# bjack205/rsLQR

Measured on AMD Instinct MI355X. Metric: LQR solves/sec (nx=12,nu=4,N=256,batch=1024 per GPU), higher is better.
Workload: dtype f64; 1 GPU; nx=12 nu=4 N=256 batch=1024 per GPU, fp64, factor+solve per step; parallelism=batch-sharded x1, no data-path collective, ranks_seen=1, flags=0, schedule=reduced-fused2

## Files before the change

### rslqr_amd/csrc/hip_context.hpp

```cpp
#pragma once
#include <hip/hip_runtime.h>

#include <cstdio>
#include <cstdlib>
#include <cstring>
#include <string>
#include <vector>

#include "ndlqr.h"
#include "ndlqr_hip.h"

#include "kernels_common.hpp"

int ndlqr_hip_fail(const char* what, hipError_t e);
struct NdlqrHipCtx;
int ndlqr_hip_ensure_F(NdlqrHipCtx* c);
#define HIP_TRY(expr)                                                  \
  do {                                                                 \
    hipError_t e_ = (expr);                                            \
    if (e_ != hipSuccess) return ndlqr_hip_fail(#expr, e_);            \
  } while (0)


enum { SLOT_LEAF = 0, SLOT_SEP, SLOT_SCHUR, SLOT_BOUNDARY, SLOT_APPLY, SLOT_BOTTOM, SLOT_UPPER, SLOT_TOP, SLOT_COUNT };

struct PendingEvent {
  int slot;
  hipEvent_t start, stop;
};

struct CapturedChain {
  hipGraphExec_t exec = nullptr;
  unsigned flags = 0;
  hipStream_t stream = nullptr;
  unsigned apply = 0;
  bool rec_complete = false;
  bool rec_compact = false;
  const char* schedule = "none";
  void reset() {
    if (exec) (void)hipGraphExecDestroy(exec);
    exec = nullptr;
  }
};

struct BufferSet {
  double* rec = nullptr;
  double* red = nullptr;
  size_t red_bytes = 0;
  double* ytop = nullptr;
  double* z = nullptr;
  double* rhs = nullptr;
  double* xfer = nullptr;
  int* tree_cnt = nullptr;
  int* h_fail = nullptr;
  hipStream_t stream = nullptr;
  hipEvent_t ev_start = nullptr, ev_stop = nullptr;
  unsigned long long rhs_gen[4] = {};
  CapturedChain graph;
  bool ready = false;
};

struct KnotSlice {
  int knot0 = 0, nknots = 0;
  unsigned blocks = 7u;
  bool valid(int N, unsigned allowed) const {
    return knot0 >= 0 && nknots > 0 && knot0 + nknots <= N && (blocks & 7u) && !(blocks & ~allowed);
  }
  size_t width(const ndlqr::Dims& u) const {
    return ((blocks & 1u) ? u.n : 0) + ((blocks & 2u) ? u.n : 0) + ((blocks & 4u) ? u.m : 0);
  }
  size_t doubles(const ndlqr::Dims& u) const { return nknots > 0 ? width(u) * nknots : (size_t)u.rows * u.N - u.m; }
};

struct NdlqrHipCtx {
  ndlqr::Dims d = {};
  ndlqr::Dims du = {};
  bool padded = false;
  double* pad_stage = nullptr;
  size_t pad_stage_cap = 0;
  int device = 0;
  unsigned flags = 0;
  bool own_stream = true;
  double* AB = nullptr;
  double* QR = nullptr;
  double* F = nullptr;
  int rowbcast = -1;
  int tree = -1;
  int fuse2 = -1;
  BufferSet set[2];
  int cur = 0;
  int latest = 0;
  int pipeline = 2;
  unsigned solve_count = 0;
  bool state_dirty = false;
  int fail_base = 0;
  int* info = nullptr;
  const char* schedule = "none";
  double* kkt_out = nullptr;
  size_t multi_cap = 0;
  double *multi_rhs = nullptr, *multi_z = nullptr, *multi_zsep = nullptr, *multi_fsum = nullptr, *multi_ytop = nullptr,
         *multi_in = nullptr, *multi_out = nullptr;
  double* sep_scratch = nullptr;
  double* h_stage[2] = {};
  bool no_top = false;
  int top_levels = 3;
  bool no_mfma = false;
  bool rec_complete = false;
  bool rec_compact = false;
  int sep_threads = 0;
  hipEvent_t ev_step[2] = {};
  unsigned step_count = 0;
  hipEvent_t ev_inputs = nullptr;
  unsigned long long rhs_latest[4] = {};
  KnotSlice sel;
  int apply_blk0 = 0, apply_nblk = 0;
  bool z_partial = false;
  bool z_invalid = false;
  int z_blk0 = 0, z_nblk = 0;
  int step_set[2] = {};
  double* h_io = nullptr;
  CapturedChain staged;
  bool timing_pending = false;
  double last_ms = 0;
  int last_failures = 0;
  bool fact_valid = false;
  double* adj_rhs = nullptr;
  double* adj_z = nullptr;
  double* adj_save = nullptr;
  double* grad_stage = nullptr;
  size_t grad_stage_cap = 0;
  unsigned long long soln_gen = 0, adj_gen = 0;
  bool inputs_replaced = false;
  double *box_lo = nullptr, *box_hi = nullptr, *box_v = nullptr, *box_y = nullptr, *box_z = nullptr, *box_qr_save = nullptr;
  double* box_rhs[2] = {};
  double* box_resid = nullptr;
  unsigned char* box_mask = nullptr;
  int *box_status = nullptr, *box_iters = nullptr, *box_word = nullptr;
  int* h_box_word = nullptr;
  bool box_shared = false, box_have_bounds = false, box_have_vy = false;
  size_t box_bstride = 0;
  bool box_fact = false;
  double box_rho = 0.0;
  unsigned box_flags = 0;
  bool box_rec_complete = false, box_rec_compact = false, box_fact_valid = false;
  const char* box_schedule = "none";
  unsigned long long box_soln_gen = 0, abox_gen = 0;
  unsigned char* abox_code = nullptr;
  double *abox_v = nullptr, *abox_y = nullptr, *abox_resid = nullptr;
  double* abox_rhs[2] = {};
  int *abox_status = nullptr, *abox_iters = nullptr, *abox_word = nullptr;
  unsigned long long factor_count = 0;
  std::vector<PendingEvent> pending;
  std::vector<hipEvent_t> event_pool;
  double slot_ms[SLOT_COUNT] = {};
  int slot_launches[SLOT_COUNT] = {};
};

static inline hipEvent_t take_event(NdlqrHipCtx* c) {
  if (!c->event_pool.empty()) {
    hipEvent_t ev = c->event_pool.back();
    c->event_pool.pop_back();
    return ev;
  }
  hipEvent_t ev = nullptr;
  (void)hipEventCreate(&ev);
  return ev;
}

struct ScopedSlot {
  NdlqrHipCtx* c;
// ... 14 lines not shown
```

### rslqr_amd/csrc/kernels_rowbcast.hpp

```cpp
#pragma once
#include "kernels_dpp.hpp"
#include "kernels_small.hpp"

namespace ndlqr {

template <int K, bool NEG>
__device__ __forceinline__ void fmac_bc4(double& a0, double& a1, double& a2, double& a3, const double x0, const double x1,
                                         const double x2, const double x3, const double y) {
  if constexpr (NEG)
    asm volatile("v_fmac_f64_dpp %0, -%4, %8 row_newbcast:%9 row_mask:0xf bank_mask:0xf\n\t"
                 "v_fmac_f64_dpp %1, -%5, %8 row_newbcast:%9 row_mask:0xf bank_mask:0xf\n\t"
                 "v_fmac_f64_dpp %2, -%6, %8 row_newbcast:%9 row_mask:0xf bank_mask:0xf\n\t"
                 "v_fmac_f64_dpp %3, -%7, %8 row_newbcast:%9 row_mask:0xf bank_mask:0xf"
                 : "+v"(a0), "+v"(a1), "+v"(a2), "+v"(a3) : "v"(x0), "v"(x1), "v"(x2), "v"(x3), "v"(y), "n"(K));
  else
    asm volatile("v_fmac_f64_dpp %0, %4, %8 row_newbcast:%9 row_mask:0xf bank_mask:0xf\n\t"
                 "v_fmac_f64_dpp %1, %5, %8 row_newbcast:%9 row_mask:0xf bank_mask:0xf\n\t"
                 "v_fmac_f64_dpp %2, %6, %8 row_newbcast:%9 row_mask:0xf bank_mask:0xf\n\t"
                 "v_fmac_f64_dpp %3, %7, %8 row_newbcast:%9 row_mask:0xf bank_mask:0xf"
                 : "+v"(a0), "+v"(a1), "+v"(a2), "+v"(a3) : "v"(x0), "v"(x1), "v"(x2), "v"(x3), "v"(y), "n"(K));
}

template <int KD, int NC, bool INIT, bool NEG = false, int NA, int NB>
__device__ __forceinline__ void rb_mul(const double (&A)[NA], double (&B)[NB], double (&out)[NC]) {
// ... 324 lines not shown
    if (hasA && rowlane) {
#pragma unroll
      for (int c = 0; c < NX; ++c)
        if (c >= i) atomicAdd(sA.DR() + c * (c + 1) / 2 + i, G[c]);
      atomicAdd(sA.gR() + i, gv);
    }
    rb_mul<NX, NX, true>(RaTt, Xb, G);
    if (hasA && hasB && rowlane) {
      if (leftchild) {
#pragma unroll
        for (int c = 0; c < NX; ++c) sB.CA()[c * NX + i] = G[c];
      } else {
        store_row<NX>(sA.CB() + i * NX, G);
      }
    }
    rb_mul<NX, NX, true>(RbTt, Xb, G);
    gv = rb_mulv<NX>(RbTt, xz);
    if (hasB && rowlane) {
#pragma unroll
      for (int c = 0; c < NX; ++c)
        if (c >= i) atomicAdd(sB.DL() + c * (c + 1) / 2 + i, G[c]);
      atomicAdd(sB.gL() + i, gv);
    }
  }
}

template <int NX>
__device__ __forceinline__ void backsub_top_body(const Dims& d, const int b, const int t,
                                                 const double* __restrict__ recs, double* __restrict__ ytop,
                                                 double* ytop_lds, const int bp, const double* zsep) {
  constexpr int NN = NX * NX, REC = 2 * NN + NX;
  const int N = d.N, K = d.K;
  const int br = bp >= 0 ? bp : b;
  for (int L = K - 1; L >= 3; --L) {
    const int T = 2 << L, nsep = N >> (L + 1);
    for (int it = t; it < nsep * NX; it += 256) {
      const int q = it / NX, r = it - q * NX;
      const int base = q * T, s = base + (T >> 1) - 1;
      const double* rc = recs + ((size_t)br * N + s) * REC;
      double acc = zsep ? zsep[((size_t)b * N + s) * NX + r] : rc[2 * NN + r];
      if (base > 0) {
        double f[NX];
        load_row<NX>(rc + r * NX, f);
        const double* y = ytop_lds + ((base - 1) >> 3) * NX;
#pragma unroll
        for (int c = 0; c < NX; ++c) acc = fma(-f[c], y[c], acc);
      }
      if (base + T < N) {
        double f[NX];
        load_row<NX>(rc + NN + r * NX, f);
        const double* y = ytop_lds + ((base + T - 1) >> 3) * NX;
#pragma unroll
        for (int c = 0; c < NX; ++c) acc = fma(-f[c], y[c], acc);
      }
      ytop_lds[(s >> 3) * NX + r] = acc;
    }
    __syncthreads();
  }
  double* out = ytop + (size_t)b * (N >> 3) * NX;
  for (int e = t; e < ((N >> 3) - 1) * NX; e += 256) out[e] = ytop_lds[e];
}

template <int NX>
__global__ __launch_bounds__(256) void rb_backsub_top(Dims d, const double* __restrict__ recs, double* __restrict__ ytop) {
  extern __shared__ double ytop_lds[];
  backsub_top_body<NX>(d, blockIdx.x, threadIdx.x, recs, ytop, ytop_lds);
}

template <int NX, int NU>
struct alignas(16) RbBacksubLds {
  static constexpr int W = NX + NU, ROWS = 2 * NX + NU, NN = NX * NX, REC = 2 * NN + NX, R0 = NX * (NX + 1) / 2;
  static constexpr int R0P = (R0 + 1) / 2 * 2;
  static constexpr int WP = RbKnot<NX, NU>::WP;
  double ab[8][NX * WP];
  double rec0[4][R0P];
  double rec1[3][REC + (REC & 1)];
  double ys[9][NX];
  double qs[8][W];
  double rs[8][ROWS];
  double dots[8][NX];
  double vs[4][NX];
};

template <int NX, int NU, bool MULTI = false>
__global__ __launch_bounds__(256) void rb_backsub(Dims d, const double* __restrict__ AB, const double* __restrict__ QR,
                                                  const double* __restrict__ rhs, const double* __restrict__ recs,
                                                  const double* __restrict__ ytop, double* __restrict__ z,
                                                  const int nprob = 0, const double* __restrict__ zsep = nullptr) {
  using Lds = RbBacksubLds<NX, NU>;
  constexpr int W = NX + NU, ROWS = 2 * NX + NU, NN = NX * NX, REC = 2 * NN + NX, KPB = 8, WP = Lds::WP;
  constexpr int R0 = Lds::R0;
  static_assert(9 * NX <= 256 && KPB * ROWS <= 256, "thread roles fit the workgroup");
  __shared__ Lds lds;
  const int N = d.N, b = blockIdx.y, first = (blockIdx.x + d.xoff) * KPB;
  const int bp = MULTI ? b % nprob : b;
  auto sep_slot = [&](int s) -> int { return s < first ? 7 : (s >= first + 7 ? 8 : s - first); };
  const int t = threadIdx.x;

  {
    const double* abm = AB + ((size_t)bp * N + first) * NX * W;
    const double* rc0 = recs + ((size_t)bp * N + first) * REC;
    constexpr int NA = KPB * NX * W / 2, IA = (NA + 255) / 256;
    constexpr bool WIDE = NX % 2 == 0 && R0 % 2 == 0;
    constexpr int G = WIDE ? 2 : 1;
    constexpr int N0 = 4 * R0 / G, I0 = (N0 + 255) / 256, N1 = 3 * REC / G, I1 = (N1 + 255) / 256;
    constexpr int NQ = KPB * W, NR = KPB * ROWS;
    static_assert(NQ <= 256 && NR <= 256, "one load per thread for the vectors");
    static_assert((KPB * NX * W) % 2 == 0, "eight knots of [A | B] are whole 16-byte words");
    constexpr int KW = NX * W / 2;
    constexpr bool BYKNOT = (NX * W) % 2 == 0 && KW % 32 == 0;
    constexpr int JA = BYKNOT ? KW / 32 : IA;
    double2 ta[JA];
    double t0[I0][G], t1[I1][G];
#pragma unroll
    for (int it = 0; it < JA; ++it) {
      if constexpr (BYKNOT) {
        ta[it] = reinterpret_cast<const double2*>(abm)[(t >> 5) * KW + (t & 31) + 32 * it];
      } else {
        const int e = t + 256 * it;
        ta[it] = reinterpret_cast<const double2*>(abm)[e < NA ? e : NA - 1];
      }
    }
#pragma unroll
    for (int it = 0; it < I0; ++it) {
      const int e = t + 256 * it, ec = e < N0 ? e : N0 - 1, j = ec / (R0 / G), w_ = ec - j * (R0 / G);
      const double* src = rc0 + (size_t)(2 * j) * REC + G * w_;
      if constexpr (WIDE) { const double2 v = *reinterpret_cast<const double2*>(src); t0[it][0] = v.x; t0[it][1] = v.y; }
      else t0[it][0] = *src;
    }
#pragma unroll
    for (int it = 0; it < I1; ++it) {
      const int e = t + 256 * it, ec = e < N1 ? e : N1 - 1, j = ec / (REC / G), w_ = ec - j * (REC / G);
      const double* src = rc0 + (size_t)(2 * j + 1) * REC + G * w_;
      if constexpr (WIDE) { const double2 v = *reinterpret_cast<const double2*>(src); t1[it][0] = v.x; t1[it][1] = v.y; }
      else t1[it][0] = *src;
    }
    const double tq = QR[((size_t)bp * N + first) * W + (t < NQ ? t : NQ - 1)];
    const double tr = rhs[((size_t)b * N + first) * ROWS + (t < NR ? t : NR - 1)];
    double tz = 0.0;
    if constexpr (MULTI) {
      const int e = t < 3 * NX ? t : 3 * NX - 1, j = e / NX;
      tz = zsep[((size_t)b * N + first + 2 * j + 1) * NX + (e - j * NX)];
    }
    double ty = 0.0;
    if (t < 2 * NX) {
      const int sx = t < NX ? first - 1 : first + 7;
      if (sx >= 0 && sx < N - 1) ty = ytop[((size_t)b * (N >> 3) + (sx >> 3)) * NX + (t < NX ? t : t - NX)];
    }
#pragma unroll
    for (int it = 0; it < JA; ++it) {
      if constexpr (BYKNOT) {
        const int w_ = 2 * ((t & 31) + 32 * it), row = w_ / W, c = w_ - row * W;
        *reinterpret_cast<double2*>(&lds.ab[t >> 5][row * WP + c]) = ta[it];
      } else {
        const int e = t + 256 * it, ec = e < NA ? e : NA - 1;
#pragma unroll
        for (int h = 0; h < 2; ++h) {
          const int ed = 2 * ec + h, kn = ed / (NX * W), w_ = ed - kn * NX * W;
          const int row = w_ / W, c = w_ - row * W;
          lds.ab[kn][row * WP + c] = h ? ta[it].y : ta[it].x;
        }
      }
    }
#pragma unroll
    for (int it = 0; it < I0; ++it) {
      const int e = t + 256 * it, ec = e < N0 ? e : N0 - 1, j = ec / (R0 / G), w_ = ec - j * (R0 / G);
#pragma unroll
      for (int h = 0; h < G; ++h) lds.rec0[j][G * w_ + h] = t0[it][h];
    }
#pragma unroll
    for (int it = 0; it < I1; ++it) {
// ... 37 lines not shown
      const double* rc = lds.rec1[q >> 1];
      double a = rc[2 * NN + r];
      if (hasA) {
#pragma unroll
        for (int c = 0; c < NX; ++c) a = fma(-rc[r * NX + c], lds.ys[slotA][c], a);
      }
      if (hasB) {
#pragma unroll
        for (int c = 0; c < NX; ++c) a = fma(-rc[NN + r * NX + c], lds.ys[slotB][c], a);
      }
      lds.ys[q][r] = a;
    }
    __syncthreads();
  }
  const bool odd_state = out_thread && (kn & 1) && rr >= NX && rr < 2 * NX;
  double dot = 0.0;
  if (odd_state) {
    if (needs_ab) dot = ab_dot(lds.ys[sep_slot(i)]);
    lds.dots[kn][rr - NX] = dot;
  }
  __syncthreads();
  if (sep_thread && l == 0) {
    const int k = s - first;
    const bool fst = s == 0;
    const double* arow = lds.ab[k] + r * WP;
    double v = 0.0;
#pragma unroll
    for (int c = 0; c < W; ++c) {
      const double wq = lds.qs[k][c];
      double zh;
      if (c < NX) zh = fst ? -lds.rs[k][c] : (lds.rs[k][NX + c] + (hasA ? lds.ys[slotA][c] : 0.0)) * wq;
      else zh = lds.rs[k][NX + c] * wq;
      v = fma(arow[c], zh, v);
    }
    const double q1 = lds.qs[k + 1][r];
    v -= lds.rs[k + 1][r] + (lds.rs[k + 1][NX + r] - lds.dots[k + 1][r]) * q1;
    lds.vs[k >> 1][r] = v;
  }
  __syncthreads();
  if (t < 64) {
    const int j = t >> 4, r15 = t & 15, rc = r15 < NX ? r15 : NX - 1;
    const double* Lp = lds.rec0[j];
    const double dinv = 1.0 / Lp[rc * (rc + 1) / 2 + rc];
    double lrow[NX], lcol[NX];
#pragma unroll
    for (int c = 0; c < NX; ++c) {
      const double lo = Lp[rc * (rc + 1) / 2 + (c < rc ? c : rc)];
      const double up = Lp[(c > rc ? c : rc) * ((c > rc ? c : rc) + 1) / 2 + rc];
      lrow[c] = (c < r15 && r15 < NX) ? lo : 0.0;
      lcol[c] = (c > r15 && r15 < NX) ? up : 0.0;
    }
    double x = lds.vs[j][rc];
    sfor<NX>([&](auto cc) {
      constexpr int c = decltype(cc)::value;
      double xs = x * dinv;
      dpp_fence(xs);
      x = fma(-lrow[c], row_bc<c>(xs), x);
    });
    x = x * dinv;
    sfor<NX>([&](auto cc) {
      constexpr int c = NX - 1 - decltype(cc)::value;
      double xs = x * dinv;
      dpp_fence(xs);
      x = fma(-lcol[c], row_bc<c>(xs), x);
    });
    if (r15 < NX) lds.ys[2 * j][r15] = x * dinv;
  }
  __syncthreads();

  if (!out_thread) return;
  const double rv = lds.rs[kn][rr];
  double out;
  const double* yi = lds.ys[sep_slot(i < N - 1 ? i : i - 1)];
  const double* yp = lds.ys[sep_slot(i > 0 ? i - 1 : 0)];
  if (needs_ab && !odd_state) dot = ab_dot(yi);
  if (lam) {
    out = (i == 0) ? fma(-QR[(size_t)bp * N * W + rr], rv, -lds.rs[0][NX + rr]) + dot : yp[rr];
  } else if (rr < 2 * NX) {
    out = (i == 0) ? -lds.rs[0][rr - NX] : (rv - dot + yp[rr - NX]) * lds.qs[kn][rr - NX];
  } else {
    out = (i == N - 1) ? rv : (rv - dot) * lds.qs[kn][rr - NX];
  }
  z[((size_t)b * N + i) * ROWS + rr] = out;
}

template <int NX>
__device__ __forceinline__ double rb_llt_solve(double x, const double (&lrow)[NX], const double (&lcol)[NX], const double dinv) {
  sfor<NX>([&](auto cc) {
    constexpr int c = decltype(cc)::value;
    double xs = x * dinv;
    dpp_fence(xs);
    x = fma(-lrow[c], row_bc<c>(xs), x);
  });
  x = x * dinv;
  sfor<NX>([&](auto cc) {
    constexpr int c = NX - 1 - decltype(cc)::value;
    double xs = x * dinv;
    dpp_fence(xs);
    x = fma(-lcol[c], row_bc<c>(xs), x);
  });
  return x * dinv;
}

template <int NX, int NU>
struct alignas(16) RbForwardLds {
  static constexpr int W = NX + NU, ROWS = 2 * NX + NU, NN = NX * NX, REC = 2 * NN + NX, R0 = NX * (NX + 1) / 2;
  static constexpr int R0P = (R0 + 1) / 2 * 2, WP = RbKnot<NX, NU>::WP;
  double ab[8][NX * WP];
  double rec0[4][R0P];
  double l1[3][NN];
  double f1[3][2 * NN];
  double qs[8][W];
  double rs[8][ROWS];
  double bt[7][NX];
  double zs[4][NX];
  double gl[7][NX], gr[7][NX];
  double outl[3][NX], outr[3][NX];
};

template <int NX, int NU, bool MULTI = false>
__global__ __launch_bounds__(256) void rb_forward(Dims d, const double* __restrict__ AB, const double* __restrict__ QR,
                                                  const double* __restrict__ rhs, double* __restrict__ recs,
                                                  double* __restrict__ fsum, const int nprob = 0,
                                                  double* __restrict__ zsep = nullptr) {
  using Lds = RbForwardLds<NX, NU>;
  constexpr int W = NX + NU, ROWS = 2 * NX + NU, NN = NX * NX, REC = 2 * NN + NX, KPB = 8, WP = Lds::WP, R0 = Lds::R0;
  static_assert(7 * NX <= 256 && KPB * ROWS <= 256 && KPB * W <= 256, "thread roles fit the workgroup");
  __shared__ Lds lds;
  const int N = d.N, b = blockIdx.y, first = blockIdx.x * KPB, t = threadIdx.x;
  const int bp = MULTI ? b % nprob : b;
  {
    const double* abm = AB + ((size_t)bp * N + first) * NX * W;
    const double* rc0 = recs + ((size_t)bp * N + first) * REC;
    constexpr bool WIDE = NX % 2 == 0 && R0 % 2 == 0 && (NX * W) % 2 == 0;
    constexpr int G = WIDE ? 2 : 1;
    constexpr int NA = KPB * NX * W / G, IA = (NA + 255) / 256;
    constexpr int N0 = 4 * R0 / G, I0 = (N0 + 255) / 256, NL = 3 * NN / G, IL = (NL + 255) / 256;
    constexpr int NF = 3 * 2 * NN / G, IF = (NF + 255) / 256;
    double ta[IA][G], t0[I0][G], tl[IL][G], tf[IF][G];
    auto ld = [](const double* src, double (&dst)[G]) {
      if constexpr (WIDE) { const double2 v = *reinterpret_cast<const double2*>(src); dst[0] = v.x; dst[1] = v.y; }
      else dst[0] = *src;
    };
#pragma unroll
    for (int it = 0; it < IA; ++it) { const int e = t + 256 * it, ec = e < NA ? e : NA - 1; ld(abm + G * ec, ta[it]); }
#pragma unroll
    for (int it = 0; it < I0; ++it) {
      const int e = t + 256 * it, ec = e < N0 ? e : N0 - 1, j = ec / (R0 / G), w_ = ec - j * (R0 / G);
      ld(rc0 + (size_t)(2 * j) * REC + G * w_, t0[it]);
    }
#pragma unroll
    for (int it = 0; it < IL; ++it) {
      const int e = t + 256 * it, ec = e < NL ? e : NL - 1, j = ec / (NN / G), w_ = ec - j * (NN / G);
      ld(rc0 + (size_t)(2 * j) * REC + rb_lrec_offset<NX>() + G * w_, tl[it]);
    }
#pragma unroll
    for (int it = 0; it < IF; ++it) {
      const int e = t + 256 * it, ec = e < NF ? e : NF - 1, j = ec / (2 * NN / G), w_ = ec - j * (2 * NN / G);
      ld(rc0 + (size_t)(2 * j + 1) * REC + G * w_, tf[it]);
    }
    const double tq = QR[((size_t)bp * N + first) * W + (t < KPB * W ? t : KPB * W - 1)];
    const double tr = rhs[((size_t)b * N + first) * ROWS + (t < KPB * ROWS ? t : KPB * ROWS - 1)];
#pragma unroll
    for (int it = 0; it < IA; ++it) {
      const int e = t + 256 * it, ec = e < NA ? e : NA - 1;
#pragma unroll
// ... 200 lines not shown
```

### rslqr_amd/csrc/launch_small.hpp

```cpp
#pragma once
#include "hip_context.hpp"
#include "kernels_leaf.hpp"
#include "kernels_small.hpp"
#include "kernels_bottom_reduced.hpp"
#include "kernels_rowbcast.hpp"

constexpr int kBottomLevels = 2;

struct SmallPlan {
  bool lean;
  int store_l;
  bool reduced;
  bool tree;
  bool compact;
  bool rowbcast;
  bool needs_F;
};

static inline unsigned apply_grid(const NdlqrHipCtx* c, const ndlqr::Dims& d) {
  return (unsigned)(c->apply_nblk > 0 ? c->apply_nblk : d.N / 8);
}
static inline ndlqr::Dims apply_dims(const NdlqrHipCtx* c, const ndlqr::Dims& d) {
  ndlqr::Dims da = d;
  if (c->apply_nblk > 0) da.xoff += c->apply_blk0;
  return da;
}

template <int NX, int NU, bool STRICT, bool KEEP>
static SmallPlan plan_small(const NdlqrHipCtx* c) {
  const ndlqr::Dims& d = c->d;
  const BufferSet& s = c->set[c->cur];
  SmallPlan p;
  p.lean = !STRICT && !KEEP && (d.K + 4) * NX <= 256;
  p.store_l = (c->flags & NDLQR_FLAG_KEEP_RECORDS) ? 1 : 0;
  p.reduced = false;
  p.tree = false;
  p.rowbcast = false;
  p.compact = false;
  if constexpr (!STRICT && !KEEP && ndlqr::P1OnMatrixCores<NX, NU>::value) {
    if (p.lean && s.red) {
      p.reduced = true;
      p.tree = s.tree_cnt && (c->tree == 1 || (c->tree < 0 && (size_t)d.batch * (d.N >> 2) <= 2048));
      p.compact = !p.tree && d.N >= 16 && 8 * (2 * NX + NU) <= 256 &&
                  sizeof(double) * (size_t)(d.N >> 3) * NX * (p.store_l ? 4 : 1) <= 160 * 1024;
      if (p.compact && p.store_l) p.store_l = 2;
      p.rowbcast = p.compact && !p.store_l && NX <= 16 && NX + NU <= 16 && (c->rowbcast == 1 || (c->rowbcast < 0 && NX <= 8));
    }
  }
  p.needs_F = !(p.reduced && p.store_l != 1);
  return p;
}

template <int NX, int NU, bool STRICT, bool KEEP>
static int launch_small(NdlqrHipCtx* c) {
  const ndlqr::Dims& d = c->d;
  BufferSet& s = c->set[c->cur];
  using Sh = ndlqr::SchurShape<NX, NU>;
  constexpr int JB = kBottomLevels;
  const SmallPlan plan = plan_small<NX, NU, STRICT, KEEP>(c);
  const bool lean = plan.lean;
  const int store_l = plan.store_l;
  c->rec_complete = !STRICT && (KEEP || (lean && store_l));
  if constexpr (!STRICT && !KEEP && ndlqr::P1OnMatrixCores<NX, NU>::value) {
    if (plan.reduced) {
      const bool tree = plan.tree;
      const bool compact = plan.compact;
      c->schedule = tree ? "reduced-tree" : (compact ? (store_l ? "reduced-compact-records" : "reduced") : "reduced-records");
      c->rec_compact = compact && store_l == 2;
      bool fuse2 = false;
      {
        ScopedSlot t(c, SLOT_BOTTOM);
        bool launched = false;
        if constexpr (NX <= 16 && NX + NU <= 16) {
          if (plan.rowbcast) {
            hipLaunchKernelGGL((ndlqr::rb_bottom<NX, NU>), dim3(d.N >> 4, d.batch), dim3(64), 0, s.stream, d, c->AB,
                               c->QR, s.rhs, s.red, s.rec, c->info);
            launched = true;
          }
        }
        fuse2 = !launched && !tree && compact && !store_l && d.N >= 16 &&
                (c->fuse2 > 0 || (c->fuse2 < 0 && NX == 12 && NU == 4));
        if (fuse2) c->schedule = "reduced-fused2";
        if (launched) {
        } else if (fuse2) {
          hipLaunchKernelGGL((ndlqr::bottom8_reduced_mc<NX, NU>), dim3(d.N >> 3, d.batch), dim3(128), 0, s.stream, d,
                             c->AB, c->QR, s.rhs, s.red, s.rec, c->info);
        } else if (tree)
          hipLaunchKernelGGL((ndlqr::bottom_reduced_mc<NX, NU, true>), dim3(d.N >> 2, d.batch), dim3(64), 0, s.stream,
                             d, c->AB, c->QR, s.rhs, s.red, s.rec, c->F, c->info, store_l, s.tree_cnt, 0);
        else if (compact)
          hipLaunchKernelGGL((ndlqr::bottom_reduced_mc<NX, NU, false, true>), dim3(d.N >> 2, d.batch), dim3(64), 0, s.stream,
                             d, c->AB, c->QR, s.rhs, s.red, s.rec, c->F, c->info, store_l, nullptr, 1);
        else
          hipLaunchKernelGGL((ndlqr::bottom_reduced_mc<NX, NU, false>), dim3(d.N >> 2, d.batch), dim3(64), 0, s.stream,
                             d, c->AB, c->QR, s.rhs, s.red, s.rec, c->F, c->info, store_l, nullptr, 0);
      }
      const int top_levels = d.K - c->top_levels >= 3 ? c->top_levels : 3;
      const int ltop = (d.K >= 5 && !c->no_top) ? d.K - top_levels : d.K;
      for (int l = fuse2 ? 3 : 2; l < ltop && !tree; ++l) {
        ScopedSlot t(c, SLOT_UPPER);
        hipLaunchKernelGGL((ndlqr::reduced_level_mc<NX, NU>), dim3(d.N >> (l + 1), d.batch), dim3(64), 0, s.stream,
                           d, l, c->AB, c->QR, s.rhs, s.red, s.rec, c->F, c->info, store_l);
      }
      const bool top_sweeps = !tree && ltop < d.K && compact &&
                              sizeof(double) * (size_t)(d.N >> 3) * NX <= 4 * sizeof(ndlqr::ReducedLds<NX, NU, false>);
      if (!tree && ltop < d.K) {
        ScopedSlot t(c, SLOT_TOP);
        const int l0 = (fuse2 && ltop < 3) ? 3 : ltop;
        hipLaunchKernelGGL((ndlqr::reduced_top_mc<NX, NU>), dim3(d.batch), dim3(256), 0, s.stream, d, l0, c->AB,
                           c->QR, s.rhs, s.red, s.rec, c->F, c->info, store_l, top_sweeps ? s.ytop : (double*)nullptr);
      }
      ScopedSlot t(c, SLOT_APPLY);
      if (compact) {
        if (!top_sweeps) {
          const size_t top_lds = sizeof(double) * (size_t)(d.N >> 3) * NX;
          if (top_lds > 64 * 1024)
            (void)hipFuncSetAttribute(reinterpret_cast<const void*>(&ndlqr::rb_backsub_top<NX>),
                                      hipFuncAttributeMaxDynamicSharedMemorySize, (int)top_lds);
          hipLaunchKernelGGL((ndlqr::rb_backsub_top<NX>), dim3(d.batch), dim3(256), top_lds, s.stream, d, s.rec, s.ytop);
        }
        hipLaunchKernelGGL((ndlqr::rb_backsub<NX, NU>), dim3(apply_grid(c, d), d.batch), dim3(256), 0, s.stream,
                           apply_dims(c, d), c->AB, c->QR, s.rhs, s.rec, s.ytop, s.z);
      } else {
        hipLaunchKernelGGL((ndlqr::backsub_small<NX, NU>), dim3(apply_grid(c, d), d.batch), dim3(256), 0, s.stream, apply_dims(c, d), c->AB,
                           c->QR, s.rhs, s.rec, s.z);
      }
      return NDLQR_OK;
    }
  }
  c->schedule = lean ? "knot-lean" : (STRICT ? "knot-strict" : "knot-keep");
  {
    ScopedSlot t(c, SLOT_BOTTOM);
    hipLaunchKernelGGL((ndlqr::bottom_small<NX, NU, STRICT, KEEP, JB>), dim3(d.N >> JB, d.batch), dim3(32 << JB), 0,
                       s.stream, d, c->AB, c->QR, s.rhs, c->F, s.z, c->info, s.rec, lean ? 1 : 0,
                       ((lean || (KEEP && !STRICT)) ? 1 : 0) | (store_l ? 2 : 0));
  }
  for (int l = JB; l < d.K; ++l) {
    ScopedSlot t(c, SLOT_UPPER);
    hipLaunchKernelGGL((ndlqr::level_small<NX, NU, STRICT, KEEP>), dim3(d.N >> (l + 1), d.batch), dim3(64), 0,
                       s.stream, d, l, c->AB, c->F, s.z, s.rec, c->info, store_l);
  }
  ScopedSlot t(c, SLOT_APPLY);
  if (lean) {
    if constexpr (!STRICT && !KEEP)
      hipLaunchKernelGGL((ndlqr::backsub_small<NX, NU>), dim3(apply_grid(c, d), d.batch), dim3(256), 0, s.stream, apply_dims(c, d), c->AB,
                         c->QR, s.rhs, s.rec, s.z);
    return NDLQR_OK;
  }
  const size_t lds = sizeof(double) * (size_t)(d.K - JB) * Sh::REC;
  hipLaunchKernelGGL((ndlqr::apply_small<NX, NU, STRICT, KEEP>), dim3(d.N / Sh::KPB, d.batch), dim3(256), lds,
                     s.stream, d, JB, c->F, s.z, s.rec);
  return NDLQR_OK;
}

template <int NX, int NU>
static void launch_rhs_records(NdlqrHipCtx* c, const double* rhs, double* z) {
  const ndlqr::Dims& d = c->d;
  BufferSet& s = c->set[c->cur];
  if constexpr (ndlqr::P1OnMatrixCores<NX, NU>::value && 8 * (2 * NX + NU) <= 256) {
    if (c->rec_compact) {
      {
        ScopedSlot t(c, SLOT_SEP);
        hipLaunchKernelGGL((ndlqr::rb_forward<NX, NU>), dim3(d.N / 8, d.batch), dim3(256), 0, s.stream, d, c->AB, c->QR,
                           rhs, s.rec, s.red);
      }
      {
        ScopedSlot t(c, SLOT_UPPER);
        const size_t lds = sizeof(double) * 4 * (size_t)(d.N >> 3) * NX;
        if (lds > 64 * 1024)
          (void)hipFuncSetAttribute(reinterpret_cast<const void*>(&ndlqr::rb_forward_top<NX, NU>),
                                    hipFuncAttributeMaxDynamicSharedMemorySize, (int)lds);
        hipLaunchKernelGGL((ndlqr::rb_forward_top<NX, NU>), dim3(d.batch), dim3(256), lds, s.stream, d, c->AB, c->QR,
                           rhs, s.rec, (const double*)s.red, s.ytop);
      }
      ScopedSlot t(c, SLOT_APPLY);
      hipLaunchKernelGGL((ndlqr::rb_backsub<NX, NU>), dim3(apply_grid(c, d), d.batch), dim3(256), 0, s.stream,
                         apply_dims(c, d), c->AB, c->QR, rhs, s.rec, s.ytop, z);
      return;
    }
  }
  {
    ScopedSlot t(c, SLOT_SEP);
    hipLaunchKernelGGL((ndlqr::rhs_forward_small<NX, NU>), dim3(d.N / 8, d.batch), dim3(64), 0, s.stream, d, c->AB,
                       c->QR, rhs, c->F, s.rec, z);
  }
  if (d.K > 3) {
    ScopedSlot t(c, SLOT_UPPER);
    const size_t lds = sizeof(double) * (size_t)(d.N / 8) * NX;
    hipLaunchKernelGGL((ndlqr::rhs_forward_upper<NX, NU>), dim3(d.batch), dim3(512), lds, s.stream, d, c->AB, c->QR,
                       rhs, c->F, s.rec, z);
  }
  {
    ScopedSlot t(c, SLOT_APPLY);
    hipLaunchKernelGGL((ndlqr::backsub_small<NX, NU>), dim3(apply_grid(c, d), d.batch), dim3(256), 0, s.stream, apply_dims(c, d), c->AB,
                       c->QR, rhs, s.rec, z);
  }
}

template <int NX, int NU>
static bool launch_multi_rhs(NdlqrHipCtx* c, const int count, const double* rhs, double* zsep, double* fsum, double* ytop,
                             double* z) {
  if constexpr (ndlqr::P1OnMatrixCores<NX, NU>::value && 8 * (2 * NX + NU) <= 256) {
    const ndlqr::Dims& d = c->d;
    BufferSet& s = c->set[c->cur];
    const size_t lds = sizeof(double) * 4 * (size_t)(d.N >> 3) * NX;
    if (lds > 160 * 1024) return false;
    if (lds > 64 * 1024)
      (void)hipFuncSetAttribute(reinterpret_cast<const void*>(&ndlqr::rb_forward_top<NX, NU, true>),
                                hipFuncAttributeMaxDynamicSharedMemorySize, (int)lds);
    hipLaunchKernelGGL((ndlqr::rb_forward<NX, NU, true>), dim3(d.N / 8, count), dim3(256), 0, s.stream, d, c->AB, c->QR, rhs,
                       s.rec, fsum, d.batch, zsep);
    hipLaunchKernelGGL((ndlqr::rb_forward_top<NX, NU, true>), dim3(count), dim3(256), lds, s.stream, d, c->AB, c->QR, rhs,
                       s.rec, (const double*)fsum, ytop, d.batch, zsep);
    hipLaunchKernelGGL((ndlqr::rb_backsub<NX, NU, true>), dim3(apply_grid(c, d), count), dim3(256), 0, s.stream,
                       apply_dims(c, d), c->AB, c->QR, rhs, (const double*)s.rec, (const double*)ytop, z, d.batch,
                       (const double*)zsep);
    return true;
  } else {
    return false;
  }
}

template <int NX, int NU>
static int launch_time_shard(NdlqrHipCtx* c, const int phase, const int g, const int G) {
  ndlqr::Dims d = c->d;
  BufferSet& bs = c->set[c->cur];
  int lg = 0;
  while ((1 << lg) < G) ++lg;
  if (G < 2 || (1 << lg) != G || g < 0 || g >= G) return NDLQR_ERR_INVALID;
  if constexpr (!ndlqr::P1OnMatrixCores<NX, NU>::value) {
    return NDLQR_ERR_INVALID;
  } else {
    const int ltop = d.K - lg;
    if (!bs.red || !bs.ytop || ltop < 4 || 8 * (2 * NX + NU) > 256 || (c->flags & ~NDLQR_FLAG_PROFILE)) return NDLQR_ERR_INVALID;
    const size_t top_lds = sizeof(double) * (size_t)(d.N >> 3) * NX;
    if (top_lds > 160 * 1024) return NDLQR_ERR_INVALID;
    if (top_lds > 64 * 1024)
      (void)hipFuncSetAttribute(reinterpret_cast<const void*>(&ndlqr::rb_backsub_top<NX>),
                                hipFuncAttributeMaxDynamicSharedMemorySize, (int)top_lds);
    constexpr size_t SLOT = ndlqr::RedSlot<NX>::SIZE;
    if (phase == 0) {
      for (int j = 1; j < G; ++j) {
        const int s = j * (d.N / G) - 1;
        double* p = bs.red + (size_t)(s >> 2) * SLOT;
        if (hipMemset2DAsync(p, sizeof(double) * (size_t)(d.N >> 2) * SLOT, 0, sizeof(double) * SLOT, (size_t)d.batch,
                             bs.stream) != hipSuccess)
          return NDLQR_ERR_NO_DEVICE;
      }
      {
        ScopedSlot t(c, SLOT_BOTTOM);
        const int cnt = (d.N >> 2) / G;
        d.xoff = g * cnt;
        hipLaunchKernelGGL((ndlqr::bottom_reduced_mc<NX, NU, false, true>), dim3(cnt, d.batch), dim3(64), 0, bs.stream, d,
                           c->AB, c->QR, bs.rhs, bs.red, bs.rec, c->F, c->info, 0, nullptr, 1);
      }
      for (int l = 2; l < ltop; ++l) {
        ScopedSlot t(c, SLOT_UPPER);
        const int cnt = (d.N >> (l + 1)) / G;
        d.xoff = g * cnt;
        hipLaunchKernelGGL((ndlqr::reduced_level_mc<NX, NU>), dim3(cnt, d.batch), dim3(64), 0, bs.stream, d, l, c->AB,
                           c->QR, bs.rhs, bs.red, bs.rec, c->F, c->info, 0);
      }
    } else {
      d.xoff = 0;
      for (int l = ltop; l < d.K; ++l) {
        ScopedSlot t(c, SLOT_TOP);
        hipLaunchKernelGGL((ndlqr::reduced_level_mc<NX, NU>), dim3(d.N >> (l + 1), d.batch), dim3(64), 0, bs.stream, d,
                           l, c->AB, c->QR, bs.rhs, bs.red, bs.rec, c->F, c->info, 0);
      }
      ScopedSlot t(c, SLOT_APPLY);
      hipLaunchKernelGGL((ndlqr::rb_backsub_top<NX>), dim3(d.batch), dim3(256), top_lds, bs.stream, d, bs.rec, bs.ytop);
      const int cnt = (d.N >> 3) / G;
      d.xoff = g * cnt;
      hipLaunchKernelGGL((ndlqr::rb_backsub<NX, NU>), dim3(cnt, d.batch), dim3(256), 0, bs.stream, d, c->AB, c->QR,
                         bs.rhs, bs.rec, bs.ytop, bs.z);
    }
    c->schedule = "reduced-time-shard";
    return NDLQR_OK;
  }
}
```

### rslqr_amd/csrc/ndlqr_hip.hip

```cpp
#include <mutex>
#include <utility>

#include "hip_context.hpp"
#include "kernels_generic.hpp"
#include "kernels_box.hpp"
#include "kernels_box_grad.hpp"
#include "kernels_grad.hpp"
#include "kernels_mfma.hpp"
#include "kernels_reduced_mfma.hpp"
#ifdef NDLQR_SINGLE_TU
#include "launch_small.hpp"
#endif


static thread_local std::string g_last_error = "";

const char* ndlqr_hip_last_error(void) { return g_last_error.c_str(); }

int ndlqr_hip_fail(const char* what, hipError_t e) {
  g_last_error = std::string(what) + ": " + hipGetErrorString(e);
  fprintf(stderr, "ndlqr_hip: %s\n", g_last_error.c_str());
  if (e == hipErrorInvalidConfiguration || e == hipErrorInvalidValue) return NDLQR_ERR_INVALID;
  return NDLQR_ERR_NO_DEVICE;
}
// ... 21 lines not shown
static const char* kSlotNames[SLOT_COUNT] = {"leaf", "separator", "schur", "schur_boundary", "apply", "bottom", "upper", "top"};

static bool has_small_instance(int nstates, int ninputs);
static void pick_pad_instance(int nstates, int ninputs, int* pn, int* pm);

static size_t bytes_AB(const ndlqr::Dims& d) { return sizeof(double) * (size_t)d.batch * d.N * d.n * d.w; }
static size_t bytes_QR(const ndlqr::Dims& d) { return sizeof(double) * (size_t)d.batch * d.N * d.w; }
static size_t bytes_z(const ndlqr::Dims& d) { return sizeof(double) * (size_t)d.batch * d.N * d.rows; }
static size_t bytes_rec(const ndlqr::Dims& d) { return sizeof(double) * (size_t)d.batch * d.N * (2 * d.n * d.n + d.n); }
static size_t bytes_F(const ndlqr::Dims& d) { return sizeof(double) * (size_t)d.batch * d.K * d.N * d.fb; }

static bool alloc_set(NdlqrHipCtx* c, BufferSet& s, bool slots) {
  const ndlqr::Dims& d = c->d;
  bool ok = hipEventCreate(&s.ev_start) == hipSuccess && hipEventCreate(&s.ev_stop) == hipSuccess &&
            hipMalloc(&s.rec, bytes_rec(d)) == hipSuccess && hipMalloc(&s.z, bytes_z(d)) == hipSuccess &&
            hipMalloc(&s.rhs, bytes_z(d)) == hipSuccess &&
            hipHostMalloc((void**)&s.h_fail, sizeof(int), hipHostMallocDefault) == hipSuccess;
  if (ok) *s.h_fail = 0;
  if (ok && slots) {
    const size_t slot_doubles = ((size_t)d.n * (d.n + 1) + 2 * (size_t)d.n * d.n + 2 * d.n + 15) / 16 * 16;
    const size_t red_bytes = sizeof(double) * (size_t)d.batch * (d.N / 4) * slot_doubles;
    const size_t cnt_bytes = sizeof(int) * (size_t)d.batch * (d.N / 4);
    ok = hipMalloc(&s.red, red_bytes) == hipSuccess && hipMemsetAsync(s.red, 0, red_bytes, s.stream) == hipSuccess &&
         hipMalloc(&s.ytop, sizeof(double) * (size_t)d.batch * (d.N / 8) * d.n) == hipSuccess &&
         hipMalloc(&s.tree_cnt, cnt_bytes) == hipSuccess && hipMemsetAsync(s.tree_cnt, 0, cnt_bytes, s.stream) == hipSuccess;
    if (ok) s.red_bytes = red_bytes;
  }
  return ok && hipMemsetAsync(s.z, 0, bytes_z(d), s.stream) == hipSuccess;
}

NdlqrHipCtx* ndlqr_hip_create(int nstates, int ninputs, int nhorizon, int batch, int device) {
  return ndlqr_hip_create_ex(nstates, ninputs, nhorizon, batch, device, 0u);
}

NdlqrHipCtx* ndlqr_hip_create_ex(int nstates, int ninputs, int nhorizon, int batch, int device, unsigned create_flags) {
  if (nstates <= 0 || ninputs <= 0 || batch <= 0 || nhorizon < 2 || (nhorizon & (nhorizon - 1))) {
    g_last_error = "invalid dimensions";
    return nullptr;
  }
  if (batch > 65535) {
    g_last_error = "batch > 65535 problems per solver: split the batch over several solvers";
    fprintf(stderr, "ndlqr_hip: %s\n", g_last_error.c_str());
    return nullptr;
  }
  int count = 0;
  hipError_t e = hipGetDeviceCount(&count);
  if (e != hipSuccess || count <= 0) {
    g_last_error = std::string("no HIP device: ") + (e != hipSuccess ? hipGetErrorString(e) : "device count is 0");
    return nullptr;
  }
  if (device < 0) {
    if (hipGetDevice(&device) != hipSuccess) device = 0;
  }
  if (device >= count) {
    g_last_error = "device index out of range";
    return nullptr;
  }
  if ((e = hipSetDevice(device)) != hipSuccess) { fail("hipSetDevice", e); return nullptr; }

  NdlqrHipCtx* c = new NdlqrHipCtx();
  ndlqr::Dims& d = c->d;
  auto set_dims = [&](ndlqr::Dims& x, int n_, int m_) {
    x.n = n_; x.m = m_; x.N = nhorizon; x.batch = batch;
    x.K = 0; while ((1 << x.K) < nhorizon) ++x.K;
    x.rows = 2 * n_ + m_; x.w = n_ + m_; x.fb = x.rows * n_; x.xoff = 0;
  };
  set_dims(c->du, nstates, ninputs);
  int pn = nstates, pm = ninputs;
  if (!has_small_instance(nstates, ninputs) && nhorizon >= 8 && !getenv("NDLQR_NO_PAD") &&
      !(create_flags & NDLQR_CREATE_NO_PAD))
    pick_pad_instance(nstates, ninputs, &pn, &pm);
  if (nstates > 128 && (nstates % 16 != 0 || (nstates + ninputs) % 4 != 0) && !getenv("NDLQR_NO_PAD") &&
      !(create_flags & NDLQR_CREATE_NO_PAD)) {
    pn = (nstates + 15) / 16 * 16;
    pm = ninputs + (4 - (pn + ninputs) % 4) % 4;
  }
  set_dims(d, pn, pm);
  c->padded = pn != nstates || pm != ninputs;
  c->device = device;
  if (getenv("NDLQR_PIPELINE")) c->pipeline = atoi(getenv("NDLQR_PIPELINE"));
  if (getenv("NDLQR_TREE")) c->tree = atoi(getenv("NDLQR_TREE")) != 0 ? 1 : 0;
  if (getenv("NDLQR_ROWBCAST")) c->rowbcast = atoi(getenv("NDLQR_ROWBCAST")) != 0 ? 1 : 0;
  if (getenv("NDLQR_FUSE2")) c->fuse2 = atoi(getenv("NDLQR_FUSE2")) != 0 ? 1 : 0;
  c->no_mfma = getenv("NDLQR_NO_MFMA") != nullptr;
  c->no_top = getenv("NDLQR_NO_TOP") != nullptr;
  if (getenv("NDLQR_TOP_LEVELS")) c->top_levels = atoi(getenv("NDLQR_TOP_LEVELS"));
  if (c->top_levels < 3 || c->top_levels > 5) c->top_levels = 3;
  if (getenv("NDLQR_SEP_THREADS")) c->sep_threads = atoi(getenv("NDLQR_SEP_THREADS"));
  BufferSet& s = c->set[0];
  bool ok = hipStreamCreateWithFlags(&s.stream, hipStreamNonBlocking) == hipSuccess &&
            hipEventCreateWithFlags(&c->ev_inputs, hipEventDisableTiming) == hipSuccess &&
            hipEventCreateWithFlags(&c->ev_step[0], hipEventDisableTiming) == hipSuccess &&
            hipEventCreateWithFlags(&c->ev_step[1], hipEventDisableTiming) == hipSuccess &&
            hipMalloc(&c->AB, bytes_AB(d)) == hipSuccess && hipMalloc(&c->QR, bytes_QR(d)) == hipSuccess &&
            hipMalloc(&c->info, sizeof(int) * ((size_t)batch + 1)) == hipSuccess &&
            alloc_set(c, s, nhorizon >= 8 && has_small_instance(d.n, d.m));
  if (ok && c->padded) {
    hipLaunchKernelGGL(ndlqr::pad_fill_generic, dim3(d.N, d.batch), dim3(128), 0, s.stream, d, c->AB, c->QR, s.rhs);
    ok = hipGetLastError() == hipSuccess;
  }
  ok = ok && hipMemsetAsync(c->info, 0, sizeof(int) * ((size_t)batch + 1), s.stream) == hipSuccess &&
       hipStreamSynchronize(s.stream) == hipSuccess;
  if (!ok) {
    fail("device allocation", hipGetLastError());
    ndlqr_hip_destroy(c);
    return nullptr;
  }
  s.ready = true;
  return c;
}

static void free_set(NdlqrHipCtx* c, int i) {
  BufferSet& s = c->set[i];
  if (s.stream) (void)hipStreamSynchronize(s.stream);
  s.graph.reset();
  (void)hipFree(s.rec); (void)hipFree(s.red); (void)hipFree(s.ytop); (void)hipFree(s.z); (void)hipFree(s.tree_cnt);
  (void)hipFree(s.rhs); (void)hipFree(s.xfer);
  if (s.h_fail) (void)hipHostFree(s.h_fail);
  if (s.ev_start) (void)hipEventDestroy(s.ev_start);
  if (s.ev_stop) (void)hipEventDestroy(s.ev_stop);
  if (s.stream && (i == 1 || c->own_stream)) (void)hipStreamDestroy(s.stream);
  s = BufferSet();
}

void ndlqr_hip_destroy(NdlqrHipCtx* c) {
  if (!c) return;
  (void)hipSetDevice(c->device);
  for (int i = 1; i >= 0; --i) free_set(c, i);
  c->staged.reset();
  if (c->h_io) (void)hipHostFree(c->h_io);
  for (auto& p : c->pending) { (void)hipEventDestroy(p.start); (void)hipEventDestroy(p.stop); }
  for (auto& ev : c->event_pool) (void)hipEventDestroy(ev);
  (void)hipFree(c->AB); (void)hipFree(c->QR); (void)hipFree(c->F); (void)hipFree(c->info);
  (void)hipFree(c->sep_scratch);
  (void)hipFree(c->multi_rhs); (void)hipFree(c->multi_z); (void)hipFree(c->multi_zsep); (void)hipFree(c->multi_fsum);
  (void)hipFree(c->multi_ytop); (void)hipFree(c->multi_in); (void)hipFree(c->multi_out);
  (void)hipFree(c->kkt_out); (void)hipFree(c->pad_stage);
  (void)hipFree(c->adj_rhs); (void)hipFree(c->adj_z); (void)hipFree(c->adj_save); (void)hipFree(c->grad_stage);
  (void)hipFree(c->box_lo); (void)hipFree(c->box_hi); (void)hipFree(c->box_v); (void)hipFree(c->box_y); (void)hipFree(c->box_z);
  (void)hipFree(c->box_qr_save); (void)hipFree(c->box_rhs[0]); (void)hipFree(c->box_rhs[1]); (void)hipFree(c->box_resid);
  (void)hipFree(c->box_mask); (void)hipFree(c->box_status); (void)hipFree(c->box_iters); (void)hipFree(c->box_word);
  (void)hipFree(c->abox_code); (void)hipFree(c->abox_v); (void)hipFree(c->abox_y); (void)hipFree(c->abox_resid);
  (void)hipFree(c->abox_rhs[0]); (void)hipFree(c->abox_rhs[1]); (void)hipFree(c->abox_status); (void)hipFree(c->abox_iters);
  (void)hipFree(c->abox_word);
  if (c->h_box_word) (void)hipHostFree(c->h_box_word);
  for (double* h : c->h_stage) if (h) (void)hipHostFree(h);
  if (c->ev_inputs) (void)hipEventDestroy(c->ev_inputs);
  for (hipEvent_t ev : c->ev_step) if (ev) (void)hipEventDestroy(ev);
  delete c;
}


static void note_solution(NdlqrHipCtx* c) {
  ++c->soln_gen;
  c->latest = c->cur;
  c->z_partial = c->apply_nblk > 0;
  c->z_invalid = false;
  c->z_blk0 = c->apply_blk0;
  c->z_nblk = c->apply_nblk;
}
static void next_solve_on_current_set(NdlqrHipCtx* c) {
  if ((c->solve_count & 1u) != (unsigned)c->cur) ++c->solve_count;
}
static int need_full_solution(const NdlqrHipCtx* c, const char* who) {
  if (c->z_invalid)
    return refuse(std::string(who) + ": the last constrained solve failed; there is no resident solution until the next solve");
// ... 2280 lines not shown
```

Measured before the change: 1.771 million solves/s.

## Add column-parallel 128-thread rb_backsub variant for small W and make it default

Adds a new backsubstitution kernel variant that assigns one thread per column across 8 knots in a 128-thread workgroup. It keeps AB rows in registers, loads the reduced records into LDS with vectorized loads, and resolves the separator ys inside waves. It replaces QR division with a Newton-refined reciprocal. The variant is selected by default when NX+NU<=16 (backsub_cols defaults to -1, which is treated as on) and can be disabled through NDLQR_BACKSUB_COLS=0. The aim is to shrink the workgroup and cut the LDS staging and sync cost of the apply stage, at the risk of lower parallelism per block and more register pressure.

```diff
diff --git a/rslqr_amd/csrc/hip_context.hpp b/rslqr_amd/csrc/hip_context.hpp
--- a/rslqr_amd/csrc/hip_context.hpp
+++ b/rslqr_amd/csrc/hip_context.hpp
@@ -86,6 +86,7 @@
   double* F = nullptr;
   int rowbcast = -1;
   int tree = -1;
+  int backsub_cols = -1;
   int fuse2 = -1;
   BufferSet set[2];
   int cur = 0;
diff --git a/rslqr_amd/csrc/kernels_rowbcast.hpp b/rslqr_amd/csrc/kernels_rowbcast.hpp
--- a/rslqr_amd/csrc/kernels_rowbcast.hpp
+++ b/rslqr_amd/csrc/kernels_rowbcast.hpp
@@ -430,11 +430,11 @@
   double vs[4][NX];
 };
 
-template <int NX, int NU, bool MULTI = false>
-__global__ __launch_bounds__(256) void rb_backsub(Dims d, const double* __restrict__ AB, const double* __restrict__ QR,
+template <int NX, int NU, bool MULTI>
+__device__ __forceinline__ void rb_backsub_staged(const Dims& d, const double* __restrict__ AB, const double* __restrict__ QR,
                                                   const double* __restrict__ rhs, const double* __restrict__ recs,
                                                   const double* __restrict__ ytop, double* __restrict__ z,
-                                                  const int nprob = 0, const double* __restrict__ zsep = nullptr) {
+                                                  const int nprob, const double* __restrict__ zsep) {
   using Lds = RbBacksubLds<NX, NU>;
   constexpr int W = NX + NU, ROWS = 2 * NX + NU, NN = NX * NX, REC = 2 * NN + NX, KPB = 8, WP = Lds::WP;
   constexpr int R0 = Lds::R0;
@@ -638,6 +638,191 @@
     out = (i == N - 1) ? rv : (rv - dot) * lds.qs[kn][rr - NX];
   }
   z[((size_t)b * N + i) * ROWS + rr] = out;
+}
+
+template <int NX>
+__device__ __forceinline__ double rb_llt_solve(double x, const double (&lrow)[NX], const double (&lcol)[NX], const double dinv);
+
+__device__ __forceinline__ double rb_rcp(const double x) {
+  double y = __builtin_amdgcn_rcp(x);
+  y = fma(fma(-x, y, 1.0), y, y);
+  return fma(fma(-x, y, 1.0), y, y);
+}
+
+constexpr int kRbBacksubColsThreads = 128;
+
+template <int NX, int NU>
+struct alignas(16) RbBacksubColsLds {
+  static constexpr int NN = NX * NX, REC = 2 * NN + NX, R0 = NX * (NX + 1) / 2;
+  static constexpr int R0P = (R0 + 1) / 2 * 2, RECP = REC + (REC & 1);
+  static constexpr int TS = 17;
+  double rec0[4][R0P];
+  union {
+    double rec1[3][RECP];
+    double prod[4][NX * TS];
+  };
+  double ys[9][NX];
+  double wv[4][NX];
+};
+
+template <int SZ>
+__device__ __forceinline__ int rec_of(const int e) { return (e >= SZ) + (e >= 2 * SZ) + (e >= 3 * SZ); }
+
+template <int NX, int NU, bool MULTI>
+__device__ __forceinline__ void rb_backsub_cols(const Dims& d, const double* __restrict__ AB, const double* __restrict__ QR,
+                                                const double* __restrict__ rhs, const double* __restrict__ recs,
+                                                const double* __restrict__ ytop, double* __restrict__ z,
+                                                const int nprob, const double* __restrict__ zsep) {
+  using Lds = RbBacksubColsLds<NX, NU>;
+  constexpr int W = NX + NU, ROWS = 2 * NX + NU, NN = NX * NX, REC = 2 * NN + NX, KPB = 8, R0 = Lds::R0, TS = Lds::TS;
+  constexpr int NT = kRbBacksubColsThreads;
+  static_assert(W <= 16 && NT == 128 && 3 * NX <= NT, "thread roles fit the workgroup");
+  __shared__ Lds lds;
+  const int N = d.N, b = blockIdx.y, first = (blockIdx.x + d.xoff) * KPB;
+  const int bp = MULTI ? b % nprob : b;
+  const int t = threadIdx.x;
+  const int odd = t >> 6, j = (t >> 4) & 3, c = t & 15;
+  const int k = 2 * j + odd, i = first + k;
+  const int cw = c < W ? c : W - 1, cx = c < NX ? c : NX - 1;
+
+  double a[NX];
+  const double* abk = AB + ((size_t)bp * N + i) * NX * W + cw;
+#pragma unroll
+  for (int r = 0; r < NX; ++r) a[r] = abk[r * W];
+  const double tq = QR[((size_t)bp * N + i) * W + cw];
+  const double* rk = rhs + ((size_t)b * N + i) * ROWS;
+  const double tl = rk[cx], tg = rk[NX + cw];
+  {
+    const double* rc0 = recs + ((size_t)bp * N + first) * REC;
+    constexpr bool WIDE = NX % 2 == 0 && R0 % 2 == 0;
+    constexpr int G = WIDE ? 2 : 1;
+    constexpr int N0 = 4 * R0 / G, I0 = (N0 + NT - 1) / NT, N1 = 3 * REC / G, I1 = (N1 + NT - 1) / NT;
+    double t0[I0][G], t1[I1][G];
+#pragma unroll
+    for (int it = 0; it < I0; ++it) {
+      const int e = t + NT * it, ec = e < N0 ? e : N0 - 1, q = rec_of<R0 / G>(ec), w_ = ec - q * (R0 / G);
+      const double* src = rc0 + (size_t)(2 * q) * REC + G * w_;
+      if constexpr (WIDE) { const double2 v = *reinterpret_cast<const double2*>(src); t0[it][0] = v.x; t0[it][1] = v.y; }
+      else t0[it][0] = *src;
+    }
+#pragma unroll
+    for (int it = 0; it < I1; ++it) {
+      const int e = t + NT * it, ec = e < N1 ? e : N1 - 1, q = rec_of<REC / G>(ec), w_ = ec - q * (REC / G);
+      const double* src = rc0 + (size_t)(2 * q + 1) * REC + G * w_;
+      if constexpr (WIDE) { const double2 v = *reinterpret_cast<const double2*>(src); t1[it][0] = v.x; t1[it][1] = v.y; }
+      else t1[it][0] = *src;
+    }
+    double tz = 0.0;
+    if constexpr (MULTI) {
+      const int e = t < 3 * NX ? t : 3 * NX - 1, q = e / NX;
+      tz = zsep[((size_t)b * N + first + 2 * q + 1) * NX + (e - q * NX)];
+    }
+    double ty = 0.0;
+    if (t < 2 * NX) {
+      const int sx = t < NX ? first - 1 : first + 7;
+      if (sx >= 0 && sx < N - 1) ty = ytop[((size_t)b * (N >> 3) + (sx >> 3)) * NX + (t < NX ? t : t - NX)];
+    }
+#pragma unroll
+    for (int it = 0; it < I0; ++it) {
+      const int e = t + NT * it, ec = e < N0 ? e : N0 - 1, q = rec_of<R0 / G>(ec), w_ = ec - q * (R0 / G);
+#pragma unroll
+      for (int h = 0; h < G; ++h) lds.rec0[q][G * w_ + h] = t0[it][h];
+    }
+#pragma unroll
+    for (int it = 0; it < I1; ++it) {
+      const int e = t + NT * it, ec = e < N1 ? e : N1 - 1, q = rec_of<REC / G>(ec), w_ = ec - q * (REC / G);
+      if (!MULTI || G * w_ < 2 * NN) {
+#pragma unroll
+        for (int h = 0; h < G; ++h) lds.rec1[q][G * w_ + h] = t1[it][h];
+      }
+    }
+    if (t < 2 * NX) lds.ys[t < NX ? 7 : 8][t < NX ? t : t - NX] = ty;
+    if constexpr (MULTI) {
+      if (t < 3 * NX) lds.rec1[t / NX][2 * NN + t % NX] = tz;
+    }
+  }
+  const double qinv = rb_rcp(tq);
+  __syncthreads();
+
+  double dot = 0.0;
+  auto ab_dot = [&](const double* y) {
+    double s = 0.0;
+#pragma unroll
+    for (int r = 0; r < NX; ++r) s = fma(a[r], y[r], s);
+    return s;
+  };
+  if (odd) {
+    auto resolve = [&](const int q, const bool hasA, const int slotA, const bool hasB, const int slotB) {
+      const double* rc = lds.rec1[q >> 1];
+      double s = rc[2 * NN + c];
+      if (hasA) {
+#pragma unroll
+        for (int e = 0; e < NX; ++e) s = fma(-rc[c * NX + e], lds.ys[slotA][e], s);
+      }
+      if (hasB) {
+#pragma unroll
+        for (int e = 0; e < NX; ++e) s = fma(-rc[NN + c * NX + e], lds.ys[slotB][e], s);
+      }
+      lds.ys[q][c] = s;
+    };
+    const bool left = first > 0, right = first + KPB < N;
+    if (j == 1 && c < NX) resolve(3, left, 7, right, 8);
+    wave_lds_sync();
+    if (j == 0 && c < NX) resolve(1, left, 7, true, 3);
+    if (j == 2 && c < NX) resolve(5, true, 3, right, 8);
+    wave_lds_sync();
+    if (i < N - 1) dot = ab_dot(lds.ys[k < 7 ? k : 8]);
+    if (c < NX) lds.wv[j][c] = tl + (tg - dot) * qinv;
+  }
+  __syncthreads();
+  if (!odd) {
+    const double ya = (i > 0 && c < NX) ? lds.ys[k > 0 ? k - 1 : 7][cx] : 0.0;
+    const double zh = (i == 0 && c < NX) ? -tl : (tg + ya) * qinv;
+    if (c < W) {
+#pragma unroll
+      for (int r = 0; r < NX; ++r) lds.prod[j][r * TS + c] = a[r] * zh;
+    }
+    wave_lds_sync();
+    const double* pr = lds.prod[j] + cx * TS;
+    double v0 = 0.0, v1 = 0.0;
+#pragma unroll
+    for (int m = 0; m + 1 < W; m += 2) { v0 += pr[m]; v1 += pr[m + 1]; }
+    if constexpr (W % 2) v0 += pr[W - 1];
+    double x = (v0 + v1) - lds.wv[j][cx];
+    const double* Lp = lds.rec0[j];
+    const double dinv = rb_rcp(Lp[cx * (cx + 1) / 2 + cx]);
+    double lrow[NX], lcol[NX];
+#pragma unroll
+    for (int e = 0; e < NX; ++e) {
+      const double lo = Lp[cx * (cx + 1) / 2 + (e < cx ? e : cx)];
+      const double up = Lp[(e > cx ? e : cx) * ((e > cx ? e : cx) + 1) / 2 + cx];
+      lrow[e] = (e < c && c < NX) ? lo : 0.0;
+      lcol[e] = (e > c && c < NX) ? up : 0.0;
+    }
+    x = rb_llt_solve<NX>(x, lrow, lcol, dinv);
+    if (c < NX) lds.ys[2 * j][c] = x;
+    wave_lds_sync();
+    dot = ab_dot(lds.ys[k]);
+  }
+  __syncthreads();
+
+  const double yp = (i > 0 && c < NX) ? lds.ys[k > 0 ? k - 1 : 7][cx] : 0.0;
+  double* zi = z + ((size_t)b * N + i) * ROWS;
+  if (c < NX) {
+    zi[c] = (i == 0) ? fma(-tq, tl, -tg) + dot : yp;
+    zi[NX + c] = (i == 0) ? -tl : (tg - dot + yp) * qinv;
+  } else if (c < W) {
+    zi[NX + c] = (i == N - 1) ? tg : (tg - dot) * qinv;
+  }
+}
+
+template <int NX, int NU, bool MULTI = false, bool COLS = false>
+__global__ __launch_bounds__(COLS ? kRbBacksubColsThreads : 256) void rb_backsub(
+    Dims d, const double* __restrict__ AB, const double* __restrict__ QR, const double* __restrict__ rhs,
+    const double* __restrict__ recs, const double* __restrict__ ytop, double* __restrict__ z, const int nprob = 0,
+    const double* __restrict__ zsep = nullptr) {
+  if constexpr (COLS) rb_backsub_cols<NX, NU, MULTI>(d, AB, QR, rhs, recs, ytop, z, nprob, zsep);
+  else rb_backsub_staged<NX, NU, MULTI>(d, AB, QR, rhs, recs, ytop, z, nprob, zsep);
 }
 
 template <int NX>
diff --git a/rslqr_amd/csrc/launch_small.hpp b/rslqr_amd/csrc/launch_small.hpp
--- a/rslqr_amd/csrc/launch_small.hpp
+++ b/rslqr_amd/csrc/launch_small.hpp
@@ -24,6 +24,17 @@
   ndlqr::Dims da = d;
   if (c->apply_nblk > 0) da.xoff += c->apply_blk0;
   return da;
+}
+
+template <int NX, int NU, bool MULTI, class... Args>
+static void launch_rb_backsub(const NdlqrHipCtx* c, const dim3 grid, hipStream_t stream, Args... args) {
+  if constexpr (NX + NU <= 16) {
+    if (c->backsub_cols != 0) {
+      hipLaunchKernelGGL((ndlqr::rb_backsub<NX, NU, MULTI, true>), grid, dim3(ndlqr::kRbBacksubColsThreads), 0, stream, args...);
+      return;
+    }
+  }
+  hipLaunchKernelGGL((ndlqr::rb_backsub<NX, NU, MULTI, false>), grid, dim3(256), 0, stream, args...);
 }
 
 template <int NX, int NU, bool STRICT, bool KEEP>
@@ -119,7 +130,7 @@
                                       hipFuncAttributeMaxDynamicSharedMemorySize, (int)top_lds);
           hipLaunchKernelGGL((ndlqr::rb_backsub_top<NX>), dim3(d.batch), dim3(256), top_lds, s.stream, d, s.rec, s.ytop);
         }
-        hipLaunchKernelGGL((ndlqr::rb_backsub<NX, NU>), dim3(apply_grid(c, d), d.batch), dim3(256), 0, s.stream,
+        launch_rb_backsub<NX, NU, false>(c, dim3(apply_grid(c, d), d.batch), s.stream,
                            apply_dims(c, d), c->AB, c->QR, s.rhs, s.rec, s.ytop, s.z);
       } else {
         hipLaunchKernelGGL((ndlqr::backsub_small<NX, NU>), dim3(apply_grid(c, d), d.batch), dim3(256), 0, s.stream, apply_dims(c, d), c->AB,
@@ -174,7 +185,7 @@
                            rhs, s.rec, (const double*)s.red, s.ytop);
       }
       ScopedSlot t(c, SLOT_APPLY);
-      hipLaunchKernelGGL((ndlqr::rb_backsub<NX, NU>), dim3(apply_grid(c, d), d.batch), dim3(256), 0, s.stream,
+      launch_rb_backsub<NX, NU, false>(c, dim3(apply_grid(c, d), d.batch), s.stream,
                          apply_dims(c, d), c->AB, c->QR, rhs, s.rec, s.ytop, z);
       return;
     }
@@ -212,7 +223,7 @@
                        s.rec, fsum, d.batch, zsep);
     hipLaunchKernelGGL((ndlqr::rb_forward_top<NX, NU, true>), dim3(count), dim3(256), lds, s.stream, d, c->AB, c->QR, rhs,
                        s.rec, (const double*)fsum, ytop, d.batch, zsep);
-    hipLaunchKernelGGL((ndlqr::rb_backsub<NX, NU, true>), dim3(apply_grid(c, d), count), dim3(256), 0, s.stream,
+    launch_rb_backsub<NX, NU, true>(c, dim3(apply_grid(c, d), count), s.stream,
                        apply_dims(c, d), c->AB, c->QR, rhs, (const double*)s.rec, (const double*)ytop, z, d.batch,
                        (const double*)zsep);
     return true;
@@ -272,7 +283,7 @@
       hipLaunchKernelGGL((ndlqr::rb_backsub_top<NX>), dim3(d.batch), dim3(256), top_lds, bs.stream, d, bs.rec, bs.ytop);
       const int cnt = (d.N >> 3) / G;
       d.xoff = g * cnt;
-      hipLaunchKernelGGL((ndlqr::rb_backsub<NX, NU>), dim3(cnt, d.batch), dim3(256), 0, bs.stream, d, c->AB, c->QR,
+      launch_rb_backsub<NX, NU, false>(c, dim3(cnt, d.batch), bs.stream, d, c->AB, c->QR,
                          bs.rhs, bs.rec, bs.ytop, bs.z);
     }
     c->schedule = "reduced-time-shard";
diff --git a/rslqr_amd/csrc/ndlqr_hip.hip b/rslqr_amd/csrc/ndlqr_hip.hip
--- a/rslqr_amd/csrc/ndlqr_hip.hip
+++ b/rslqr_amd/csrc/ndlqr_hip.hip
@@ -127,6 +127,7 @@
   if (getenv("NDLQR_TREE")) c->tree = atoi(getenv("NDLQR_TREE")) != 0 ? 1 : 0;
   if (getenv("NDLQR_ROWBCAST")) c->rowbcast = atoi(getenv("NDLQR_ROWBCAST")) != 0 ? 1 : 0;
   if (getenv("NDLQR_FUSE2")) c->fuse2 = atoi(getenv("NDLQR_FUSE2")) != 0 ? 1 : 0;
+  if (getenv("NDLQR_BACKSUB_COLS")) c->backsub_cols = atoi(getenv("NDLQR_BACKSUB_COLS")) != 0 ? 1 : 0;
   c->no_mfma = getenv("NDLQR_NO_MFMA") != nullptr;
   c->no_top = getenv("NDLQR_NO_TOP") != nullptr;
   if (getenv("NDLQR_TOP_LEVELS")) c->top_levels = atoi(getenv("NDLQR_TOP_LEVELS"));
```

Measured after the change: 1.885 million solves/s, median of 6. 6.5% higher.
